# dmmiller612/sparktorch

Measured on AMD Instinct MI355X. Metric: samples_per_sec, higher is better.
Workload: dtype bf16; 1 GPU; model=mnist_mlp_784x256x256x10, global_batch=2097152, parallelism=dp1, optimizer=fused_adam, loss=cross_entropy_fused, hipgraph=False

## Files before the change

sparktorch_amd/ops/csrc/bindings.cpp:

```cpp

#include <torch/extension.h>

#include <c10/hip/HIPStream.h>
#include <hip/hip_runtime.h>

#include <cstdint>

typedef uint16_t bf16raw;

extern "C" {
hipError_t launch_fused_adam(float*, const float*, float*, float*, int64_t, float, float, float,
                             float, float, float, float, float, int, const int*, hipStream_t);
hipError_t launch_increment_i32(int*, hipStream_t);
hipError_t launch_fused_sgd(float*, const float*, float*, int64_t, float, float, float, float,
                            float, int, int, int, hipStream_t);
hipError_t launch_relu_bwd(const bf16raw*, const bf16raw*, bf16raw*, int64_t, hipStream_t);
hipError_t launch_bias_grad(const bf16raw*, float*, int, int, float*, int,
                            hipStream_t);
hipError_t launch_small_wgrad(const bf16raw*, const bf16raw*, float*, float*, int, int64_t, int,
                              int, hipStream_t);
hipError_t launch_pad_nhwc(const bf16raw*, bf16raw*, int, int, int, int, int, hipStream_t);
hipError_t launch_s2d_stem(const bf16raw*, bf16raw*, int, int, int, int, hipStream_t);
hipError_t launch_flip_w2d(const bf16raw*, bf16raw*, int, int, int, hipStream_t);
hipError_t launch_conv_implicit_fwd(const bf16raw*, const bf16raw*, const float*, bf16raw*, int,
                                    int, int, int, int, int, int, int, int, int, int, int, int,
                                    hipStream_t);
hipError_t launch_conv_implicit_wgrad(const bf16raw*, const bf16raw*, float*, int, int, int, int,
                                      int, int, int, int, int, int, float*, int, int,
                                      hipStream_t);
int conv_implicit_wgrad_slices(int, int);
hipError_t launch_cast_f64_f32(const double*, float*, int64_t, hipStream_t);
hipError_t launch_cast_f64_bf16(const double*, bf16raw*, int64_t, hipStream_t);
hipError_t launch_cast_f32_bf16(const float*, bf16raw*, int64_t, hipStream_t);
hipError_t launch_ce_fused(const bf16raw*, const int64_t*, float*, bf16raw*, int, int,
                           hipStream_t);
hipError_t launch_mse_fused(const bf16raw*, const bf16raw*, float*, bf16raw*, int64_t,
                            hipStream_t);
hipError_t launch_gemm_bf16(const void*, const void*, int, float*, bf16raw*, const float*, int,
                            int, int, int64_t, int64_t, int64_t, int64_t, int, int, float*, int,
                            hipStream_t);
hipError_t launch_gemm_bf16_mask(const void*, const void*, int, float*, bf16raw*, const float*,
                                 int, int, int, int64_t, int64_t, int64_t, int64_t, int, int,
                                 float*, int, const bf16raw*, hipStream_t);
int head_bwd_supported(int, int);
int linear_wgrad_stream_supported(int, int, int64_t);
int linear_wgrad_stream_can_run(int, int, int64_t);
hipError_t launch_linear_wgrad_stream(const bf16raw*, const bf16raw*, float*, float*, int64_t, int,
                                      int, int, int, hipStream_t);
int linear_fwd_stream_supported(int, int, int64_t);
int64_t linear_fwd_stream_min_rows();
hipError_t launch_linear_stream(const bf16raw*, const bf16raw*, bf16raw*, const float*,
                                const bf16raw*, int64_t, int, int, int, int, int, hipStream_t);
hipError_t launch_sample_gather(const void*, int, const void*, int, void*, void*, int*, const int*,
                                uint32_t, int64_t, int, int, int, int, hipStream_t);
hipError_t launch_head_bwd(const bf16raw*, const bf16raw*, const bf16raw*, bf16raw*, float*,
                           float*, int, int, int, int, int, hipStream_t);
hipError_t launch_bn_stats(const bf16raw*, float*, float*, float*, float*, float*, float*, int,
                           int, int64_t, float, float, int, hipStream_t);
hipError_t launch_bn_apply(const bf16raw*, const bf16raw*, bf16raw*, const float*, const float*,
                           const float*, const float*, int, int64_t, int64_t, int, hipStream_t);
hipError_t launch_bn_bwd_reduce(const bf16raw*, const bf16raw*, const bf16raw*, const float*,
                                const float*, float*, float*, int, int, int64_t, int,
                                hipStream_t);
hipError_t launch_bn_bwd_dx(const bf16raw*, const bf16raw*, const bf16raw*, const float*,
                            const float*, const float*, const float*, const float*, bf16raw*,
                            int, int64_t, int64_t, float, int, hipStream_t);
hipError_t launch_add_relu(const bf16raw*, const bf16raw*, bf16raw*, int64_t, hipStream_t);
hipError_t launch_maxpool_gen_fwd(const bf16raw*, bf16raw*, uint8_t*, int64_t, int, int, int,
                                  int, int, int, int, hipStream_t);
hipError_t launch_maxpool_gen_bwd(const bf16raw*, const uint8_t*, bf16raw*, int64_t, int, int,
                                  int, int, int, int, int, hipStream_t);
hipError_t launch_gap_fwd(const bf16raw*, bf16raw*, int64_t, int64_t, hipStream_t);
hipError_t launch_gap_bwd(const bf16raw*, bf16raw*, int64_t, int64_t, hipStream_t);
hipError_t launch_im2col_nhwc(const bf16raw*, bf16raw*, int, int, int, int, int, int, int, int,
                              int, int, int, int, int, hipStream_t);
hipError_t launch_col2im_nhwc(const bf16raw*, bf16raw*, int, int, int, int, int, int, int, int,
                              int, int, int, int, int, hipStream_t);
hipError_t launch_maxpool_nhwc_fwd(const bf16raw*, bf16raw*, uint8_t*, int, int, int, int, int,
                                   int, int, int, int, hipStream_t);
hipError_t launch_maxpool_nhwc_bwd(const bf16raw*, const uint8_t*, bf16raw*, int, int, int, int,
                                   int, int, int, int, int, hipStream_t);
hipError_t launch_gap_nhwc_fwd(const bf16raw*, bf16raw*, int, int, int64_t, hipStream_t);
hipError_t launch_gap_nhwc_bwd(const bf16raw*, bf16raw*, int, int, int64_t, hipStream_t);
hipError_t launch_bn_stats_nhwc(const bf16raw*, float*, float*, float*, float*, float*, float*,
                                int64_t, int, float, float, int, float*, int, hipStream_t);
hipError_t launch_bn_apply_nhwc(const bf16raw*, const bf16raw*, bf16raw*, const float*,
                                const float*, const float*, const float*, int, int64_t, int,
                                hipStream_t);
hipError_t launch_bn_bwd_reduce_nhwc(const bf16raw*, const bf16raw*, const bf16raw*,
// ... 417 lines not shown
    ip = idx_out->data_ptr<int>();
  }
  CHECK_HIP(launch_sample_gather(x.data_ptr(), (int)x.element_size(), yp, y_es, xb.data_ptr(), ybp,
                                 ip, step_dev.data_ptr<int>(), (uint32_t)(seed & 0xFFFFFFFFLL), n,
                                 (int)k, (int)F, (int)L, head_num_cus(), cur_stream()));
}

at::Tensor linear_head_bwd(at::Tensor dz_out, at::Tensor w, at::Tensor y_in, at::Tensor dw,
                           c10::optional<at::Tensor> db, int64_t max_blocks) {
  check_gpu_contig(dz_out, at::kBFloat16, "dz_out");
  check_gpu_contig(w, at::kBFloat16, "w");
  check_gpu_contig(y_in, at::kBFloat16, "y_in");
  check_gpu_contig(dw, at::kFloat, "dw");
  TORCH_CHECK(dz_out.dim() == 2 && w.dim() == 2 && y_in.dim() == 2);
  int64_t B = dz_out.size(0), C = dz_out.size(1), H = w.size(1);
  TORCH_CHECK(B >= 1 && B < (1LL << 31) && w.size(0) == C && y_in.size(0) == B &&
                  y_in.size(1) == H && dw.size(0) == C && dw.size(1) == H,
              "shape mismatch");
  TORCH_CHECK(head_bwd_ok(C, H), "linear_head_bwd: unsupported (C, H); use the per-layer route");
  float* dbp = nullptr;
  if (db.has_value()) {
    check_gpu_contig(*db, at::kFloat, "db");
    TORCH_CHECK(db->numel() == C);
    dbp = db->data_ptr<float>();
  }
  auto dz_in = at::empty({B, H}, y_in.options());
  TORCH_CHECK(((uintptr_t)y_in.data_ptr() & 15) == 0 && ((uintptr_t)dz_in.data_ptr() & 15) == 0,
              "linear_head_bwd wants 16-byte aligned activations");
  CHECK_HIP(launch_head_bwd((const bf16raw*)dz_out.data_ptr(), (const bf16raw*)w.data_ptr(),
                            (const bf16raw*)y_in.data_ptr(), (bf16raw*)dz_in.data_ptr(),
                            dw.data_ptr<float>(), dbp, (int)B, (int)C, (int)H, (int)max_blocks,
                            head_num_cus(), cur_stream()));
  return dz_in;
}


static bool small_wgrad_path(int64_t M, int64_t N, int64_t K) {
  return (K & 7) == 0 && N * K <= 2048 && N <= 64 && K <= 512 && M >= 65536;
}
static int small_wgrad_slices(int64_t M) {
  int64_t s = M / 4096;
  return (int)(s < 256 ? 256 : (s > 2048 ? 2048 : s));
}

at::Tensor linear_wgrad(at::Tensor dz, at::Tensor x, int64_t splitk) {
  check_gpu_contig(dz, at::kBFloat16, "dz");
  check_gpu_contig(x, at::kBFloat16, "x");
  int64_t B = dz.size(0), N = dz.size(1), K = x.size(1);
  TORCH_CHECK(x.size(0) == B, "shape mismatch");
  if (small_wgrad_path(B, N, K)) {
    auto dw = at::zeros({N, K}, x.options().dtype(at::kFloat));
    int S = small_wgrad_slices(B);
    auto scratch = at::empty({(int64_t)S * N * K}, x.options().dtype(at::kFloat));
    CHECK_HIP(launch_small_wgrad((const bf16raw*)dz.data_ptr(), (const bf16raw*)x.data_ptr(),
                                 dw.data_ptr<float>(), scratch.data_ptr<float>(), S, B, (int)N,
                                 (int)K, cur_stream()));
    return dw;
  }
  at::Tensor dw = splitk > 1 ? at::zeros({N, K}, x.options().dtype(at::kFloat))
                             : at::empty({N, K}, x.options().dtype(at::kFloat));
  CHECK_HIP(launch_gemm_bf16(dz.data_ptr(), x.data_ptr(),  0, dw.data_ptr<float>(),
                             nullptr, nullptr, (int)N, (int)K, (int)B,
                              1,  N,  K,  1, 0, (int)splitk,
                             nullptr, -1, cur_stream()));
  return dw;
}
// ... 527 lines not shown
  m.def("conv_implicit_wgrad", &conv_implicit_wgrad, "implicit-GEMM s1 conv weight grad",
        py::arg("dz"), py::arg("xP"), py::arg("KH"), py::arg("KW"), py::arg("splitk"),
        py::arg("slab"), py::arg("OHo") = -1, py::arg("OWo") = -1,
        py::arg("SH") = 1, py::arg("SW") = 1);
  m.def("cast_f64_f32", &cast_f64_f32);
  m.def("cast_f64_bf16", &cast_f64_bf16, "one-pass device Vector pack cast");
  m.def("cast_f32_bf16", &cast_f32_bf16);
  m.def("ce_fused", &ce_fused, "cross-entropy fwd+bwd fused");
  m.def("mse_fused", &mse_fused, "mse fwd+bwd fused");
  m.def("linear_fwd", &linear_fwd, "Y = X W^T (+bias)(+relu), MFMA", py::arg("x"), py::arg("w"),
        py::arg("bias"), py::arg("relu"), py::arg("allow_stream") = true);
  m.def("linear_dgrad", &linear_dgrad, "dX = dZ W, MFMA", py::arg("dz"), py::arg("w"),
        py::arg("allow_stream") = true);
  m.def("linear_fwd_stream_supported", &linear_fwd_stream_ok,
        "can the full-N streaming Linear kernel compute C[M, N] from a K-deep reduction",
        py::arg("N"), py::arg("K"), py::arg("M"));
  m.def("linear_fwd_stream_min_rows", &linear_stream_min_rows,
        "M from which linear_fwd / linear_dgrad(_relu) route supported shapes to it");
  m.def("set_linear_stream_min_rows", &set_linear_stream_min_rows,
        "override that M (tests); negative restores the measured one; returns the old setting",
        py::arg("rows"));
  m.def("linear_fwd_stream", &linear_fwd_stream,
        "Y = X W^T (+bias)(+relu) through the full-N streaming kernel, any M", py::arg("x"),
        py::arg("w"), py::arg("bias"), py::arg("relu"));
  m.def("linear_dgrad_stream", &linear_dgrad_stream,
        "dX = dZ W (* (y_prev > 0)) through the full-N streaming kernel, any M", py::arg("dz"),
        py::arg("w"), py::arg("y_prev") = py::none());
  m.def("linear_dgrad_relu", &linear_dgrad_relu, "dX = (dZ W) * (y_prev > 0), MFMA",
        py::arg("dz"), py::arg("w"), py::arg("y_prev"), py::arg("allow_stream") = true);
  m.def("head_bwd_supported", &head_bwd_ok, "does the one-pass head backward serve (C, H)");
  m.def("linear_head_bwd", &linear_head_bwd, "one-pass dz_in/dW/db of a small head on a ReLU layer",
        py::arg("dz_out"), py::arg("w"), py::arg("y_in"), py::arg("dw"), py::arg("db"),
        py::arg("max_blocks") = 0);
  m.def("linear_wgrad_stream_supported", &linear_wgrad_stream_ok,
        "is (No, Ki) at batch B routed to the batch-streaming wgrad");
  m.def("linear_wgrad_stream_can_run", &linear_wgrad_stream_runs,
        "can the batch-streaming wgrad compute (No, Ki, B) at all");
  m.def("linear_wgrad_stream", &linear_wgrad_stream,
        "dW (+ db) accumulated by the persistent batch-streaming kernel", py::arg("dz"),
        py::arg("x"), py::arg("dw"), py::arg("db") = py::none(), py::arg("max_blocks") = 0);
  m.def("linear_wgrad", &linear_wgrad, "dW = dZ^T X, MFMA split-K");
  m.def("linear_wgrad_into", &linear_wgrad_into, "dW accumulated into grad view");
  m.def("linear_wgrad_bias_into", &linear_wgrad_bias_into, "dW + db in one MFMA launch");
  m.def("bias_grad_into", &bias_grad_into, "db accumulated into grad view");
  m.def("matmul_bf16", &matmul_bf16, "generic bf16 MFMA GEMM");
  m.def("im2col", &im2col, "NCHW -> implicit-GEMM col matrix");
  m.def("col2im", &col2im, "col gradient -> NCHW input gradient");
  m.def("maxpool_fwd", &maxpool_fwd, "max_pool2d (kernel==stride) + argmax");
  m.def("maxpool_bwd", &maxpool_bwd, "max_pool2d backward scatter");
  m.def("dropout_apply", &dropout_apply, "counter-based dropout / dropout2d");
  m.def("bn_stats", &bn_stats, "BatchNorm2d training stats (mean, invstd) + running update");
  m.def("bn_apply", &bn_apply, "BN normalize+affine (+residual)(+relu)");
  m.def("bn_bwd_reduce", &bn_bwd_reduce, "BN backward: dbeta/dgamma accumulated in-place");
  m.def("bn_bwd_dx", &bn_bwd_dx, "BN backward input gradient");
  m.def("add_relu", &add_relu, "out = relu(a+b) (residual join)");
  m.def("maxpool_gen_fwd", &maxpool_gen_fwd, "general max_pool2d (stride/pad) + argmax");
  m.def("maxpool_gen_bwd", &maxpool_gen_bwd, "general max_pool2d backward (gather)");
  m.def("gap_fwd", &gap_fwd, "global average pool [B,C,H,W]->[B,C]");
  m.def("gap_bwd", &gap_bwd, "global average pool backward");
  m.def("im2col_nhwc", &im2col_nhwc, "BHWC -> implicit-GEMM col (vectorized over C)");
  m.def("col2im_nhwc", &col2im_nhwc, "col gradient -> BHWC input gradient");
  m.def("maxpool_nhwc_fwd", &maxpool_nhwc_fwd, "NHWC max_pool2d (stride/pad) + argmax");
  m.def("maxpool_nhwc_bwd", &maxpool_nhwc_bwd, "NHWC max_pool2d backward (gather)");
  m.def("gap_nhwc_fwd", &gap_nhwc_fwd, "NHWC global average pool -> [B,C]");
  m.def("gap_nhwc_bwd", &gap_nhwc_bwd, "NHWC global average pool backward");
  m.def("bn_stats_nhwc", &bn_stats_nhwc, "NHWC BN training stats + running update");
// ... 5 lines not shown
```

sparktorch_amd/ops/csrc/common.h:

```cpp
#pragma once

#include <hip/hip_runtime.h>

#include <cstdint>

#define WAVE 64

typedef uint16_t bf16raw;

__device__ __forceinline__ float bf16_to_f32(bf16raw h) {
  union {
    uint32_t u;
    float f;
  } c;
  c.u = ((uint32_t)h) << 16;
  return c.f;
}

__device__ __forceinline__ bf16raw f32_to_bf16(float f) {
  union {
    float f;
    uint32_t u;
  } c;
  c.f = f;
  uint32_t u = c.u;
  uint32_t rounding = 0x7fff + ((u >> 16) & 1);
  u += rounding;
  return (bf16raw)(u >> 16);
}

typedef float floatx4 __attribute__((ext_vector_type(4)));
typedef float floatx16 __attribute__((ext_vector_type(16)));
typedef short shortx8 __attribute__((ext_vector_type(8)));
typedef short shortx4 __attribute__((ext_vector_type(4)));

__host__ __device__ __forceinline__ int64_t ceil_div_i64(int64_t a, int64_t b) {
  return (a + b - 1) / b;
}

__host__ __device__ __forceinline__ uint32_t hash_u32(uint32_t a, uint32_t seed) {
  uint32_t h = a * 0x9E3779B9u + seed;
  h ^= h >> 16;
  h *= 0x85EBCA6Bu;
  h ^= h >> 13;
  h *= 0xC2B2AE35u;
  h ^= h >> 16;
  return h;
}

#define HIP_CHECK_LAUNCH()                                         \
  do {                                                             \
    hipError_t err_ = hipGetLastError();                           \
    if (err_ != hipSuccess) return err_;                           \
  } while (0)
```

sparktorch_amd/ops/csrc/head_bwd.hip:

```cpp

#include "common.h"

typedef shortx8 hfrag_t;

#define HEAD_THREADS 256
#define HEAD_CPAD 16

__host__ __device__ constexpr int head_rows(int H) { return H <= 256 ? 64 : 32; }

template <bool TR>
__device__ __forceinline__ hfrag_t head_tr_frag(const bf16raw* __restrict__ img, int stride,
                                                int xm, int rb, int q, int l15, int col0) {
  hfrag_t f;
  if (TR) {
    const int col = col0 + 4 * (l15 & 3);
#pragma unroll
    for (int jh = 0; jh < 2; ++jh) {
      const int row = rb + jh * 16 + q * 4 + (l15 >> 2);
      const bf16raw* p = img + row * stride + ((((col >> 3) ^ (row & xm)) << 3) | (col & 7));
      shortx4 v = __builtin_amdgcn_ds_read_tr16_b64_v4i16(
          (__attribute__((address_space(3))) shortx4*)p);
#pragma unroll
      for (int j = 0; j < 4; ++j) f[jh * 4 + j] = v[j];
    }
  } else {
    const int col = col0 + l15;
#pragma unroll
    for (int i = 0; i < 8; ++i) {
      const int row = rb + (i >> 2) * 16 + q * 4 + (i & 3);
      f[i] = (short)img[row * stride + ((((col >> 3) ^ (row & xm)) << 3) | (col & 7))];
    }
  }
  return f;
}

template <int H, bool TR>
__global__ __launch_bounds__(HEAD_THREADS, 2) void head_bwd_kernel(
    const bf16raw* __restrict__ dz_out, const bf16raw* __restrict__ w,
    const bf16raw* __restrict__ y_in, bf16raw* __restrict__ dz_in, float* __restrict__ dw,
    float* __restrict__ db, int B, int C) {
  constexpr int ROWS = head_rows(H);
  constexpr int SLOTS = H / 8;
  constexpr int XM = (SLOTS % 16 == 0) ? 15 : 7;
  constexpr int NP = H / 32;
  constexpr int PW = (NP + 3) / 4;
  constexpr int NCH = ROWS * H * 2 / 1024;
  constexpr int EPT = ROWS * HEAD_CPAD / HEAD_THREADS;
  static_assert(H % 64 == 0 && H <= 512, "unsupported H");

  __shared__ __attribute__((aligned(16))) bf16raw ys[2][ROWS * H];
  __shared__ __attribute__((aligned(16))) bf16raw dzs[2][ROWS * HEAD_CPAD];

  const int t = threadIdx.x;
  const int wid = t >> 6, lane = t & 63;
  const int l15 = lane & 15, q = lane >> 4;
  const int ntiles = (B + ROWS - 1) / ROWS;

  hfrag_t wf[PW][2];
#pragma unroll
  for (int pi = 0; pi < PW; ++pi) {
    const int p = wid + pi * 4;
#pragma unroll
    for (int e = 0; e < 2; ++e) {
      const int h = p * 32 + (l15 >> 2) * 8 + e * 4 + (l15 & 3);
#pragma unroll
      for (int i = 0; i < 8; ++i) {
        const int c = q * 8 + i;
        wf[pi][e][i] = (p < NP && c < C) ? (short)w[c * H + h] : (short)0;
      }
    }
  }
  hfrag_t ones;
#pragma unroll
  for (int i = 0; i < 8; ++i) ones[i] = (short)0x3F80;

  floatx4 accw[PW][2] = {};
  floatx4 accb = {0.f, 0.f, 0.f, 0.f};

  const int zrow = (t * EPT) / HEAD_CPAD, zc0 = (t * EPT) % HEAD_CPAD;
  bf16raw zr[EPT];
  auto load_dz = [&](int tile) {
    const int64_t gr = (int64_t)tile * ROWS + zrow;
#pragma unroll
    for (int j = 0; j < EPT; ++j)
      zr[j] = (gr < B && zc0 + j < C) ? dz_out[gr * C + zc0 + j] : (bf16raw)0;
  };
  auto write_dz = [&](int b) {
#pragma unroll
    for (int j = 0; j < EPT; ++j) dzs[b][zrow * HEAD_CPAD + zc0 + j] = zr[j];
  };
  auto dma_y = [&](int b, int tile) {
#pragma unroll
    for (int c = wid; c < NCH; c += 4) {
      const int o = c * 1024 + lane * 16;
      const int row = o / (H * 2);
      const int slot = ((o % (H * 2)) >> 4) ^ (row & XM);
      int64_t gr = (int64_t)tile * ROWS + row;
      if (gr > B - 1) gr = B - 1;
      const bf16raw* g = y_in + gr * H + slot * 8;
      __builtin_amdgcn_global_load_lds(
          (const __attribute__((address_space(1))) unsigned int*)g,
          (__attribute__((address_space(3))) unsigned int*)(ys[b] + c * 512), 16, 0, 0);
    }
  };

  int tile = blockIdx.x;
  int buf = 0;
  if (tile < ntiles) {
    dma_y(0, tile);
    load_dz(tile);
    write_dz(0);
  }
  for (; tile < ntiles; tile += gridDim.x) {
    __syncthreads();
    const int next = tile + gridDim.x;
    if (next < ntiles) {
      load_dz(next);
      dma_y(buf ^ 1, next);
    }
    const bf16raw* yb = ys[buf];
    const bf16raw* zb = dzs[buf];
    const int64_t row0 = (int64_t)tile * ROWS;

#pragma unroll
    for (int rf = 0; rf < ROWS / 16; ++rf) {
      const int row = rf * 16 + l15;
      hfrag_t bz = {};
      if (q < 2) bz = *(const hfrag_t*)&zb[row * HEAD_CPAD + q * 8];
#pragma unroll
      for (int pi = 0; pi < PW; ++pi) {
        const int p = wid + pi * 4;
        if (p < NP) {
          floatx4 z = {0.f, 0.f, 0.f, 0.f};
          floatx4 a0 = __builtin_amdgcn_mfma_f32_16x16x32_bf16(wf[pi][0], bz, z, 0, 0, 0);
          floatx4 a1 = __builtin_amdgcn_mfma_f32_16x16x32_bf16(wf[pi][1], bz, z, 0, 0, 0);
          const int slot = p * 4 + q;
          const shortx8 mk = *(const shortx8*)&yb[row * H + ((slot ^ (row & XM)) << 3)];
          shortx8 out;
#pragma unroll
          for (int j = 0; j < 4; ++j) {
            out[j] = bf16_to_f32((bf16raw)mk[j]) > 0.f ? (short)f32_to_bf16(a0[j]) : (short)0;
            out[4 + j] =
                bf16_to_f32((bf16raw)mk[4 + j]) > 0.f ? (short)f32_to_bf16(a1[j]) : (short)0;
          }
          if (row0 + row < B) *(shortx8*)(dz_in + (row0 + row) * H + slot * 8) = out;
        }
      }
    }

#pragma unroll
    for (int ks = 0; ks < ROWS / 32; ++ks) {
      const hfrag_t bz = head_tr_frag<TR>(zb, HEAD_CPAD, 0, ks * 32, q, l15, 0);
      if (wid == 0)
        accb = __builtin_amdgcn_mfma_f32_16x16x32_bf16(ones, bz, accb, 0, 0, 0);
#pragma unroll
      for (int pi = 0; pi < PW; ++pi) {
        const int p = wid + pi * 4;
        if (p < NP) {
#pragma unroll
          for (int e = 0; e < 2; ++e) {
            const hfrag_t ay = head_tr_frag<TR>(yb, H, XM, ks * 32, q, l15, p * 32 + e * 16);
            accw[pi][e] = __builtin_amdgcn_mfma_f32_16x16x32_bf16(ay, bz, accw[pi][e], 0, 0, 0);
          }
        }
      }
    }

    if (next < ntiles) write_dz(buf ^ 1);
    buf ^= 1;
  }

  if (l15 < C) {
#pragma unroll
    for (int pi = 0; pi < PW; ++pi) {
      const int p = wid + pi * 4;
      if (p < NP) {
#pragma unroll
        for (int e = 0; e < 2; ++e)
#pragma unroll
          for (int r = 0; r < 4; ++r)
            atomicAdd(dw + l15 * H + p * 32 + e * 16 + q * 4 + r, accw[pi][e][r]);
      }
    }
    if (db != nullptr && wid == 0 && q == 0) atomicAdd(db + l15, accb[0]);
  }
}

extern "C" int head_bwd_supported(int C, int H) {
  return C >= 1 && C <= HEAD_CPAD && (H == 64 || H == 128 || H == 256 || H == 512);
}

extern "C" hipError_t launch_head_bwd(const bf16raw* dz_out, const bf16raw* w,
                                      const bf16raw* y_in, bf16raw* dz_in, float* dw, float* db,
                                      int B, int C, int H, int max_blocks, int num_cus,
                                      hipStream_t stream) {
  if (!head_bwd_supported(C, H) || B < 1) return hipErrorInvalidValue;
  const int ntiles = (B + head_rows(H) - 1) / head_rows(H);
  int grid = 2 * (num_cus > 0 ? num_cus : 256);
  if (max_blocks > 0 && grid > max_blocks) grid = max_blocks;
  if (grid > ntiles) grid = ntiles;
#define HEAD_LAUNCH(HH)                                                                     \
  head_bwd_kernel<HH, true><<<dim3(grid), dim3(HEAD_THREADS), 0, stream>>>(dz_out, w, y_in, \
                                                                            dz_in, dw, db, B, C)
  switch (H) {
    case 64: HEAD_LAUNCH(64); break;
    case 128: HEAD_LAUNCH(128); break;
    case 256: HEAD_LAUNCH(256); break;
    default: HEAD_LAUNCH(512); break;
  }
#undef HEAD_LAUNCH
  HIP_CHECK_LAUNCH();
  return hipSuccess;
}
```

sparktorch_amd/ops/csrc/loss.hip:

```cpp

#include "common.h"


__global__ void ce_fused_kernel(const bf16raw* __restrict__ logits,
                                const int64_t* __restrict__ tgt, float* __restrict__ loss_out,
                                bf16raw* __restrict__ dlogits, int B, int C, float inv_B) {
  int64_t b = (int64_t)blockIdx.x * blockDim.x + threadIdx.x;
  float my_loss = 0.f;
  if (b < B) {
    const bf16raw* row = logits + b * C;
    bf16raw* drow = dlogits + b * C;
    float mx = -1e30f;
    for (int c = 0; c < C; ++c) mx = fmaxf(mx, bf16_to_f32(row[c]));
    float se = 0.f;
    for (int c = 0; c < C; ++c) se += __expf(bf16_to_f32(row[c]) - mx);
    float lse = __logf(se) + mx;
    int64_t t = tgt[b];
    my_loss = (lse - bf16_to_f32(row[t])) * inv_B;
    float inv_se = 1.f / se;
    for (int c = 0; c < C; ++c) {
      float p = __expf(bf16_to_f32(row[c]) - mx) * inv_se;
      if (c == (int)t) p -= 1.f;
      drow[c] = f32_to_bf16(p * inv_B);
    }
// ... 9 lines not shown
}

__global__ void ce_fused_wave_kernel(const bf16raw* __restrict__ logits,
                                     const int64_t* __restrict__ tgt,
                                     float* __restrict__ loss_out,
                                     bf16raw* __restrict__ dlogits, int B, int C, float inv_B) {
  int wave = threadIdx.x >> 6;
  int lane = threadIdx.x & 63;
  int64_t b = (int64_t)blockIdx.x * 4 + wave;
  if (b >= B) return;
  const bf16raw* row = logits + b * C;
  bf16raw* drow = dlogits + b * C;
  float mx = -1e30f;
  for (int c = lane; c < C; c += 64) mx = fmaxf(mx, bf16_to_f32(row[c]));
  for (int off = 32; off; off >>= 1) mx = fmaxf(mx, __shfl_xor(mx, off, 64));
  float se = 0.f;
  for (int c = lane; c < C; c += 64) se += __expf(bf16_to_f32(row[c]) - mx);
  for (int off = 32; off; off >>= 1) se += __shfl_xor(se, off, 64);
  int64_t t = tgt[b];
  float inv_se = 1.f / se;
  for (int c = lane; c < C; c += 64) {
    float p = __expf(bf16_to_f32(row[c]) - mx) * inv_se;
    if (c == (int)t) p -= 1.f;
    drow[c] = f32_to_bf16(p * inv_B);
  }
  if (lane == 0) {
    float my_loss = (__logf(se) + mx - bf16_to_f32(row[t])) * inv_B;
    atomicAdd(loss_out, my_loss);
  }
}

extern "C" hipError_t launch_ce_fused(const bf16raw* logits, const int64_t* tgt, float* loss_out,
                                      bf16raw* dlogits, int B, int C, hipStream_t stream) {
  if (C >= 128 || B <= 2048) {
    int grid = (int)ceil_div_i64(B, 4);
    ce_fused_wave_kernel<<<grid, 256, 0, stream>>>(logits, tgt, loss_out, dlogits, B, C,
                                                   1.0f / B);
  } else {
    int block = 256;
    int grid = (int)ceil_div_i64(B, block);
    ce_fused_kernel<<<grid, block, 0, stream>>>(logits, tgt, loss_out, dlogits, B, C, 1.0f / B);
  }
  HIP_CHECK_LAUNCH();
  return hipSuccess;
}


__global__ void mse_fused_kernel(const bf16raw* __restrict__ pred,
                                 const bf16raw* __restrict__ target, float* __restrict__ loss_out,
                                 bf16raw* __restrict__ dpred, int64_t n, float inv_n) {
  int64_t i = (int64_t)blockIdx.x * blockDim.x + threadIdx.x;
  int64_t stride = (int64_t)gridDim.x * blockDim.x;
  float my = 0.f;
  for (int64_t k = i; k < n; k += stride) {
    float d = bf16_to_f32(pred[k]) - bf16_to_f32(target[k]);
    my += d * d * inv_n;
    dpred[k] = f32_to_bf16(2.f * d * inv_n);
  }
  __shared__ float red[256];
  red[threadIdx.x] = my;
  __syncthreads();
  for (int s = blockDim.x / 2; s > 0; s >>= 1) {
    if (threadIdx.x < s) red[threadIdx.x] += red[threadIdx.x + s];
    __syncthreads();
  }
  if (threadIdx.x == 0 && red[0] != 0.f) atomicAdd(loss_out, red[0]);
}
// ... 11 lines not shown
```

sparktorch_amd/ops/functional.py:

```python

from __future__ import annotations

from typing import Optional

import torch
import torch.nn.functional as F

from sparktorch_amd import ops


def _choose_splitk(batch: int, n_out: int, k_in: int) -> int:
    base = -(-n_out // 128) * (-(-k_in) // 128)
    want = max(1, 2048 // max(1, base))
    max_by_rows = max(1, batch // 512)
    return int(min(want, max_by_rows, 512))


_WGRAD_STREAM = True
_WGRAD_STREAM_MIN_BATCH = None


def _wgrad_stream_ok(ext, dz: torch.Tensor, x: torch.Tensor) -> bool:
    if not _WGRAD_STREAM or dz.data_ptr() % 16 or x.data_ptr() % 16:
        return False
# ... 177 lines not shown
        b_direct = need_b and b_notify is not None and b.grad is not None
        dw_t = w.grad if w_direct else torch.zeros_like(w, dtype=torch.float32)
        db_t = None
        if need_b:
            db_t = b.grad if b_direct else torch.zeros_like(b, dtype=torch.float32)
        dz_prev = ext.linear_head_bwd(dz, wb, xin, dw_t, db_t, 0)
        if w_direct:
            w_notify()
        if b_direct:
            b_notify()
        return dz_prev, (None if w_direct else dw_t), (None if b_direct else db_t)


def hip_mlp_chain(x: torch.Tensor, layers) -> torch.Tensor:
    if x.is_cuda:
        if x.dtype != torch.bfloat16:
            x = x.to(torch.bfloat16)
        if not x.is_contiguous():
            x = x.contiguous()
        lead = x.shape[:-1]
        flat = []
        for w, b, _ in layers:
            flat += [w, b]
        relus = tuple(bool(r) for _, _, r in layers)
        y = _MLPChainFn.apply(x.reshape(-1, x.shape[-1]), relus, *flat)
        return y.view(*lead, y.shape[-1]) if x.dim() != 2 else y
    for w, b, relu in layers:
        x = F.linear(x, w, b)
        if relu:
            x = F.relu(x)
    return x


class _Conv2dFn(torch.autograd.Function):

    @staticmethod
    def forward(ctx, x, w, b, stride, padding, relu):
        ext = ops.ext()
        B, CI, H, W = x.shape
        CO, _, KH, KW = w.shape
        sh, sw = stride
        ph, pw = padding
        HO = (H + 2 * ph - KH) // sh + 1
        WO = (W + 2 * pw - KW) // sw + 1
        col = ext.im2col(x, KH, KW, sh, sw, ph, pw)
        w2d = w.reshape(CO, CI * KH * KW).contiguous()
        y2d = ext.linear_fwd(col, w2d, b, relu, allow_stream=False)
        ctx.save_for_backward(col, w2d, y2d)
        ctx.meta = (B, CI, H, W, CO, KH, KW, sh, sw, ph, pw, HO, WO, relu, b is not None)
        ctx.w_ref, ctx.b_ref = w, b
        return y2d.view(B, HO, WO, CO).permute(0, 3, 1, 2).contiguous()

    @staticmethod
    def backward(ctx, dy):
        ext = ops.ext()
        col, w2d, y2d = ctx.saved_tensors
        B, CI, H, W, CO, KH, KW, sh, sw, ph, pw, HO, WO, relu, has_bias = ctx.meta
        dy2d = dy.permute(0, 2, 3, 1).reshape(B * HO * WO, CO).contiguous()
        if dy2d.dtype != torch.bfloat16:
            dy2d = dy2d.to(torch.bfloat16)
        dz = ext.relu_bwd(dy2d, y2d) if relu else dy2d

        w, b = ctx.w_ref, ctx.b_ref
        dw = db = None
        sk = _choose_splitk(dz.shape[0], CO, col.shape[1])
        w_notify = getattr(w, "_bucket_notify", None)
# ... 607 lines not shown
```

sparktorch_amd/ops/modules.py:

```python

from __future__ import annotations

from typing import Optional

import torch
import torch.nn as nn

from sparktorch_amd.ops.functional import (
    hip_add_relu,
    hip_batch_norm2d,
    hip_batch_norm2d_nhwc,
    hip_conv2d,
    hip_conv2d_nhwc,
    hip_cross_entropy,
    hip_dropout,
    hip_global_avg_pool,
    hip_global_avg_pool_nhwc,
    hip_linear,
    hip_max_pool2d,
    hip_max_pool2d_nhwc,
    hip_mlp_chain,
    hip_relu,
    hip_mse,
)


class HipLinear(nn.Module):

    def __init__(self, in_features: int, out_features: int, bias: bool = True,
                 activation: Optional[str] = None):
        super().__init__()
        self.in_features = in_features
        self.out_features = out_features
        self.weight = nn.Parameter(torch.empty(out_features, in_features))
        self.bias = nn.Parameter(torch.zeros(out_features)) if bias else None
        self.activation = activation
        nn.init.kaiming_uniform_(self.weight, a=5 ** 0.5)

    @classmethod
    def from_linear(cls, lin: nn.Linear, activation: Optional[str] = None) -> "HipLinear":
        m = cls.__new__(cls)
        nn.Module.__init__(m)
        m.in_features = lin.in_features
        m.out_features = lin.out_features
        m.weight = lin.weight
        m.bias = lin.bias
        m.activation = activation
        return m

    def forward(self, x: torch.Tensor) -> torch.Tensor:
        return hip_linear(x, self.weight, self.bias, relu=self.activation == "relu")

    def extra_repr(self) -> str:
        return "in=%d, out=%d, act=%s" % (self.in_features, self.out_features, self.activation)
# ... 191 lines not shown
        self.fc = HipLinear(512, num_classes)

    def forward(self, x):
        if x.is_cuda and x.dtype != torch.bfloat16:
            x = x.to(torch.bfloat16)
        if x.dim() == 2:
            x = x.view(-1, 3, 224, 224)
        if self.layout == "nhwc":
            x = x.permute(0, 2, 3, 1).contiguous()
        x = self.bn1(self.conv1(x))
        x = self.maxpool(x)
        x = self.layers(x)
        return self.fc(self.gap(x))


class HipCrossEntropy(nn.Module):
    def forward(self, logits, target):
        return hip_cross_entropy(logits, target)


class HipMSE(nn.Module):
    def forward(self, pred, target):
        return hip_mse(pred, target)


class MnistMLPFused(nn.Module):

    def __init__(self, in_dim: int = 784, hidden: int = 256, classes: int = 10):
        super().__init__()
        self.fc1 = HipLinear(in_dim, hidden, activation="relu")
        self.fc2 = HipLinear(hidden, hidden, activation="relu")
        self.fc3 = HipLinear(hidden, classes, activation=None)

    def forward(self, x: torch.Tensor) -> torch.Tensor:
        return hip_mlp_chain(x, [(fc.weight, fc.bias, fc.activation == "relu")
                                 for fc in (self.fc1, self.fc2, self.fc3)])


def convert_model_for_mi355x(model: nn.Module) -> nn.Module:
    for name, child in model.named_children():
        cname = type(child).__name__
        if cname in ("Linear",) or isinstance(child, nn.Linear):
            setattr(model, name, HipLinear.from_linear(child))
        elif cname in ("Conv2d",) or isinstance(child, nn.Conv2d):
            try:
                setattr(model, name, HipConv2d.from_conv2d(child))
            except (ValueError, AttributeError):
                pass
        elif cname == "MaxPool2d" or isinstance(child, nn.MaxPool2d):
            ks, st, pd = child.kernel_size, child.stride, child.padding
            if isinstance(ks, int) and isinstance(st, (int, type(None))) and isinstance(pd, int) \
                    and child.dilation == 1 and not child.ceil_mode:
                setattr(model, name, HipMaxPool2d(ks, stride=st, padding=pd))
        elif cname == "BatchNorm2d" or isinstance(child, nn.BatchNorm2d):
            try:
                setattr(model, name, HipBatchNorm2d.from_batchnorm(child))
            except (ValueError, AttributeError):
                pass
        elif cname == "AdaptiveAvgPool2d" and child.output_size in (1, (1, 1)):
            setattr(model, name, HipGlobalAvgPool(keepdim=True))
        elif cname == "Dropout2d":
            setattr(model, name, HipDropout(p=child.p, channel_wise=True))
        elif cname == "Dropout":
            setattr(model, name, HipDropout(p=child.p, channel_wise=False))
        else:
            convert_model_for_mi355x(child)
    return model


# ... 8 lines not shown
```

sparktorch_amd/parallel/sync.py:

```python

from __future__ import annotations

import random
from typing import Any, Iterable, List, Optional

import numpy as np
import torch
import torch.distributed as dist

from sparktorch_amd.compat.barrier import get_barrier_context
from sparktorch_amd.parallel.buckets import FlatBuckets
from sparktorch_amd.parallel.rendezvous import (
    cleanup_stale_process_group,
    init_process_group_from_barrier,
    pick_device,
)
from sparktorch_amd.utils.data import handle_features, handle_features_device
from sparktorch_amd.utils.early_stopper import EarlyStopping
from sparktorch_amd.utils.sampling import DeviceMinibatchSampler
from sparktorch_amd.utils.trace import StepMetrics, trace_range
from sparktorch_amd.utils.serialize import (
    load_base_torch,
    load_torch_model,
    serialize_torch_obj,
# ... 39 lines not shown
                convert_model_for_mi355x,
            )

            self.model = convert_model_for_mi355x(self.model)
            self.criterion = convert_criterion_for_mi355x(self.criterion)
        self.world_size = (
            world_size
            if world_size is not None
            else (dist.get_world_size() if dist.is_initialized() else 1)
        )

        self.buckets = FlatBuckets(
            list(self.model.parameters()), bucket_cap_mb=bucket_cap_mb, world_size=self.world_size
        )
        self.buckets.register_hooks()

        from sparktorch_amd.ops.optim import fused_optimizer_for

        self.optimizer = fused_optimizer_for(torch_optimizer, self.buckets)
        self._torch_opt = None
        if self.optimizer is None:
            self._torch_opt = type(torch_optimizer)(
                self.model.parameters(), **torch_optimizer.defaults
            )

        self._graph = None
        self._graph_inputs = None
        self._sampled_graph = None
        self.compile_mode = compile_mode
        if compile_mode and compile_mode not in ("hipgraph",):
            self.model = torch.compile(self.model, mode=compile_mode)

    def _forward_backward(self, x: torch.Tensor, y: torch.Tensor) -> torch.Tensor:
        pred = self.model(x)
        loss = compute_loss(self.criterion, pred, y)
        loss.backward()
        return loss

    def train_step(self, x: torch.Tensor, y: torch.Tensor) -> float:
        if self.compile_mode == "hipgraph" and x.is_cuda:
            return self._train_step_graphed(x, y)
        self.buckets.zero_grad()
        loss = self._forward_backward(x, y)
        if self.optimizer is not None:
            self.buckets.finalize(average=False)
            self.optimizer.step(grad_scale=1.0 / self.world_size)
        else:
            self.buckets.finalize(average=True)
            self._torch_opt.step()
        return float(loss.detach())

    def _train_step_graphed(self, x: torch.Tensor, y: torch.Tensor) -> float:
        key = (tuple(x.shape), tuple(y.shape) if y is not None else None)
        if self._graph is None or self._graph_inputs[0] != key:
            if self.world_size > 1:
                raise RuntimeError(
                    "compileMode='hipgraph' currently supports world_size==1 "
                    "(collectives are not graph-captured)"
                )
            static_x = x.clone()
            static_y = y.clone() if y is not None else None
            snap_params = [b.flat_param.clone() for b in self.buckets.buckets]
            snap_buffers = {k: v.clone() for k, v in self.model.named_buffers()}
            snap_opt = None
            if self.optimizer is not None:
                sd = getattr(self.optimizer, "step_dev", None)
# ... 301 lines not shown
```

Measured before the change: 390.6 million samples/s.

## Fuse MLP head forward, cross-entropy and head backward into one kernel

Adds a head_ce kernel that computes head logits with MFMA, softmax cross-entropy, the loss reduction and the dlogits-driven backward (dz_in, dW, db) in a single pass over the last hidden activations. The MLP training step routes through a manual, autograd-free forward/backward chain when the criterion is HipCrossEntropy. This avoids writing and re-reading the logits and dlogits tensors and cuts separate kernel launches and autograd overhead. In exchange the code is more complex, uses inline barriers, and sums the loss with float atomics, so it is order-dependent.

After: 425.8 million samples/s, median of 6. 9.0% higher.

```diff
diff --git a/sparktorch_amd/ops/csrc/bindings.cpp b/sparktorch_amd/ops/csrc/bindings.cpp
--- a/sparktorch_amd/ops/csrc/bindings.cpp
+++ b/sparktorch_amd/ops/csrc/bindings.cpp
@@ -55,6 +55,8 @@
                                 uint32_t, int64_t, int, int, int, int, hipStream_t);
 hipError_t launch_head_bwd(const bf16raw*, const bf16raw*, const bf16raw*, bf16raw*, float*,
                            float*, int, int, int, int, int, hipStream_t);
+hipError_t launch_head_ce(const bf16raw*, const float*, const bf16raw*, const int64_t*, bf16raw*,
+                          float*, float*, float*, bf16raw*, int, int, int, int, int, hipStream_t);
 hipError_t launch_bn_stats(const bf16raw*, float*, float*, float*, float*, float*, float*, int,
                            int, int64_t, float, float, int, hipStream_t);
 hipError_t launch_bn_apply(const bf16raw*, const bf16raw*, bf16raw*, const float*, const float*,
@@ -538,6 +540,45 @@
                             dw.data_ptr<float>(), dbp, (int)B, (int)C, (int)H, (int)max_blocks,
                             head_num_cus(), cur_stream()));
   return dz_in;
+}
+
+std::tuple<at::Tensor, at::Tensor, at::Tensor> linear_head_ce(
+    at::Tensor y_in, at::Tensor w, c10::optional<at::Tensor> bias, at::Tensor target,
+    at::Tensor dw, c10::optional<at::Tensor> db, bool want_logits, int64_t max_blocks) {
+  check_gpu_contig(y_in, at::kBFloat16, "y_in");
+  check_gpu_contig(w, at::kBFloat16, "w");
+  check_gpu_contig(target, at::kLong, "target");
+  check_gpu_contig(dw, at::kFloat, "dw");
+  TORCH_CHECK(y_in.dim() == 2 && w.dim() == 2 && target.dim() == 1);
+  int64_t B = y_in.size(0), H = y_in.size(1), C = w.size(0);
+  TORCH_CHECK(B >= 1 && B < (1LL << 31) && w.size(1) == H && target.size(0) == B &&
+                  dw.dim() == 2 && dw.size(0) == C && dw.size(1) == H,
+              "shape mismatch");
+  TORCH_CHECK(head_bwd_ok(C, H), "linear_head_ce: unsupported (C, H); use the three-step route");
+  const float* bp = nullptr;
+  if (bias.has_value()) {
+    check_gpu_contig(*bias, at::kFloat, "bias");
+    TORCH_CHECK(bias->numel() == C);
+    bp = bias->data_ptr<float>();
+  }
+  float* dbp = nullptr;
+  if (db.has_value()) {
+    check_gpu_contig(*db, at::kFloat, "db");
+    TORCH_CHECK(db->numel() == C);
+    dbp = db->data_ptr<float>();
+  }
+  auto loss = at::empty({}, y_in.options().dtype(at::kFloat));
+  auto dz_in = at::empty({B, H}, y_in.options());
+  auto logits = want_logits ? at::empty({B, C}, y_in.options()) : at::empty({0}, y_in.options());
+  TORCH_CHECK(((uintptr_t)y_in.data_ptr() & 15) == 0 && ((uintptr_t)dz_in.data_ptr() & 15) == 0 &&
+                  ((uintptr_t)w.data_ptr() & 15) == 0,
+              "linear_head_ce wants 16-byte aligned activations and weights");
+  CHECK_HIP(launch_head_ce((const bf16raw*)w.data_ptr(), bp, (const bf16raw*)y_in.data_ptr(),
+                           target.data_ptr<int64_t>(), (bf16raw*)dz_in.data_ptr(),
+                           dw.data_ptr<float>(), dbp, loss.data_ptr<float>(),
+                           want_logits ? (bf16raw*)logits.data_ptr() : nullptr, (int)B, (int)C,
+                           (int)H, (int)max_blocks, head_num_cus(), cur_stream()));
+  return {loss, dz_in, logits};
 }
 
 
@@ -1131,6 +1172,10 @@
   m.def("linear_head_bwd", &linear_head_bwd, "one-pass dz_in/dW/db of a small head on a ReLU layer",
         py::arg("dz_out"), py::arg("w"), py::arg("y_in"), py::arg("dw"), py::arg("db"),
         py::arg("max_blocks") = 0);
+  m.def("linear_head_ce", &linear_head_ce,
+        "head forward + cross-entropy + one-pass head backward: (loss, dz_in, logits)",
+        py::arg("y_in"), py::arg("w"), py::arg("bias"), py::arg("target"), py::arg("dw"),
+        py::arg("db"), py::arg("want_logits") = false, py::arg("max_blocks") = 0);
   m.def("linear_wgrad_stream_supported", &linear_wgrad_stream_ok,
         "is (No, Ki) at batch B routed to the batch-streaming wgrad");
   m.def("linear_wgrad_stream_can_run", &linear_wgrad_stream_runs,
diff --git a/sparktorch_amd/ops/csrc/common.h b/sparktorch_amd/ops/csrc/common.h
--- a/sparktorch_amd/ops/csrc/common.h
+++ b/sparktorch_amd/ops/csrc/common.h
@@ -48,7 +48,9 @@
   return h;
 }
 
-#define HIP_CHECK_LAUNCH()                                         \
+#define CE_WAVE_MAX_B 2048
+
+#define HIP_CHECK_LAUNCH()                                        \
   do {                                                             \
     hipError_t err_ = hipGetLastError();                           \
     if (err_ != hipSuccess) return err_;                           \
diff --git a/sparktorch_amd/ops/csrc/head_bwd.hip b/sparktorch_amd/ops/csrc/head_bwd.hip
--- a/sparktorch_amd/ops/csrc/head_bwd.hip
+++ b/sparktorch_amd/ops/csrc/head_bwd.hip
@@ -34,11 +34,13 @@
   return f;
 }
 
-template <int H, bool TR>
-__global__ __launch_bounds__(HEAD_THREADS, 2) void head_bwd_kernel(
+template <int H, bool TR, bool CE>
+__device__ __forceinline__ void head_tiles(
     const bf16raw* __restrict__ dz_out, const bf16raw* __restrict__ w,
     const bf16raw* __restrict__ y_in, bf16raw* __restrict__ dz_in, float* __restrict__ dw,
-    float* __restrict__ db, int B, int C) {
+    float* __restrict__ db, int B, int C, const float* __restrict__ bias,
+    const int64_t* __restrict__ tgt, float* __restrict__ loss, bf16raw* __restrict__ logits_out,
+    float inv_B) {
   constexpr int ROWS = head_rows(H);
   constexpr int SLOTS = H / 8;
   constexpr int XM = (SLOTS % 16 == 0) ? 15 : 7;
@@ -49,7 +51,7 @@
   static_assert(H % 64 == 0 && H <= 512, "unsupported H");
 
   __shared__ __attribute__((aligned(16))) bf16raw ys[2][ROWS * H];
-  __shared__ __attribute__((aligned(16))) bf16raw dzs[2][ROWS * HEAD_CPAD];
+  __shared__ __attribute__((aligned(16))) bf16raw dzs[CE ? 1 : 2][ROWS * HEAD_CPAD];
 
   const int t = threadIdx.x;
   const int wid = t >> 6, lane = t & 63;
@@ -76,6 +78,25 @@
 
   floatx4 accw[PW][2] = {};
   floatx4 accb = {0.f, 0.f, 0.f, 0.f};
+
+  hfrag_t wk[CE ? H / 32 : 1];
+  float bias_c = 0.f, lsum = 0.f;
+  int tg[4] = {0, 0, 0, 0};
+  if (CE) {
+#pragma unroll
+    for (int ks = 0; ks < H / 32; ++ks) {
+      wk[ks] = hfrag_t{};
+      if (l15 < C) wk[ks] = *(const hfrag_t*)&w[l15 * H + ks * 32 + q * 8];
+    }
+    if (bias != nullptr && l15 < C) bias_c = bias[l15];
+  }
+  auto load_tgt = [&](int tile) {
+    if (wid < ROWS / 16) {
+      const int64_t gr = (int64_t)tile * ROWS + wid * 16 + q * 4;
+#pragma unroll
+      for (int r = 0; r < 4; ++r) tg[r] = (gr + r < B) ? (int)tgt[gr + r] : 0;
+    }
+  };
 
   const int zrow = (t * EPT) / HEAD_CPAD, zc0 = (t * EPT) % HEAD_CPAD;
   bf16raw zr[EPT];
@@ -108,19 +129,101 @@
   int buf = 0;
   if (tile < ntiles) {
     dma_y(0, tile);
-    load_dz(tile);
-    write_dz(0);
+    if (CE) {
+      load_tgt(tile);
+    } else {
+      load_dz(tile);
+      write_dz(0);
+    }
   }
   for (; tile < ntiles; tile += gridDim.x) {
-    __syncthreads();
+    if (CE)
+      asm volatile("s_waitcnt vmcnt(0) lgkmcnt(0)\n\ts_barrier" ::: "memory");
+    else
+      __syncthreads();
     const int next = tile + gridDim.x;
-    if (next < ntiles) {
+    const bf16raw* yb = ys[buf];
+    bf16raw* zb = dzs[CE ? 0 : buf];
+    const int64_t row0 = (int64_t)tile * ROWS;
+    if (CE) {
+      int tc[4];
+#pragma unroll
+      for (int r = 0; r < 4; ++r) tc[r] = tg[r];
+      constexpr bool EARLY = H <= 256;
+      const bool fwd_wave = wid < ROWS / 16;
+      const int arow = wid * 16 + l15;
+      hfrag_t ay[H / 32];
+      if (EARLY && fwd_wave) {
+#pragma unroll
+        for (int ks = 0; ks < H / 32; ++ks)
+          ay[ks] = *(const hfrag_t*)&yb[arow * H + (((ks * 4 + q) ^ (arow & XM)) << 3)];
+      }
+      if (next < ntiles) {
+        dma_y(buf ^ 1, next);
+        load_tgt(next);
+      }
+      if (fwd_wave) {
+#pragma clang fp reassociate(off)
+        floatx4 lg = {0.f, 0.f, 0.f, 0.f};
+#pragma unroll
+        for (int ks = 0; ks < H / 32; ++ks) {
+          if (!EARLY)
+            ay[ks] = *(const hfrag_t*)&yb[arow * H + (((ks * 4 + q) ^ (arow & XM)) << 3)];
+          lg = __builtin_amdgcn_mfma_f32_16x16x32_bf16(ay[ks], wk[ks], lg, 0, 0, 0);
+        }
+        constexpr int RG = H <= 256 ? 4 : 1;
+#pragma unroll
+        for (int r0 = 0; r0 < 4; r0 += RG) {
+          bf16raw xb[RG];
+          float x[RG], mx[RG], e[RG], se[RG];
+#pragma unroll
+          for (int j = 0; j < RG; ++j) {
+            xb[j] = f32_to_bf16(bias != nullptr ? lg[r0 + j] + bias_c : lg[r0 + j]);
+            x[j] = bf16_to_f32(xb[j]);
+            mx[j] = l15 < C ? fmaxf(-1e30f, x[j]) : -1e30f;
+          }
+#pragma unroll
+          for (int off = 8; off; off >>= 1)
+#pragma unroll
+            for (int j = 0; j < RG; ++j) mx[j] = fmaxf(mx[j], __shfl_xor(mx[j], off, 16));
+#pragma unroll
+          for (int j = 0; j < RG; ++j) e[j] = l15 < C ? __expf(x[j] - mx[j]) : 0.f;
+          if (B <= CE_WAVE_MAX_B) {
+#pragma unroll
+            for (int j = 0; j < RG; ++j) se[j] = e[j];
+#pragma unroll
+            for (int off = 8; off; off >>= 1)
+#pragma unroll
+              for (int j = 0; j < RG; ++j) se[j] += __shfl_xor(se[j], off, 16);
+          } else {
+#pragma unroll
+            for (int j = 0; j < RG; ++j) se[j] = 0.f;
+            for (int c = 0; c < C; ++c)
+#pragma unroll
+              for (int j = 0; j < RG; ++j) se[j] += __shfl(e[j], c, 16);
+          }
+#pragma unroll
+          for (int j = 0; j < RG; ++j) {
+            const int r = r0 + j;
+            const int lrow = wid * 16 + q * 4 + r;
+            const bool live = row0 + lrow < B;
+            const float xt = __shfl(x[j], tc[r] & 15, 16);
+            const float inv_se = 1.f / se[j];
+            const float p =
+                l15 == tc[r] ? __builtin_fmaf(e[j], inv_se, -1.f) : e[j] * inv_se;
+            zb[lrow * HEAD_CPAD + l15] =
+                (live && l15 < C) ? f32_to_bf16(p * inv_B) : (bf16raw)0;
+            if (live && l15 == 0) lsum += (__logf(se[j]) + mx[j] - xt) * inv_B;
+            if (logits_out != nullptr && live && l15 < C)
+              logits_out[(row0 + lrow) * C + l15] = xb[j];
+          }
+        }
+      }
+      asm volatile("s_waitcnt lgkmcnt(0)\n\ts_barrier" ::: "memory");
+    } else if (next < ntiles) {
       load_dz(next);
       dma_y(buf ^ 1, next);
     }
-    const bf16raw* yb = ys[buf];
-    const bf16raw* zb = dzs[buf];
-    const int64_t row0 = (int64_t)tile * ROWS;
 
 #pragma unroll
     for (int rf = 0; rf < ROWS / 16; ++rf) {
@@ -166,8 +269,22 @@
       }
     }
 
-    if (next < ntiles) write_dz(buf ^ 1);
+    if (!CE && next < ntiles) write_dz(buf ^ 1);
     buf ^= 1;
+  }
+
+  if (CE) {
+    __shared__ float lred[HEAD_THREADS / 64];
+#pragma unroll
+    for (int off = 32; off; off >>= 1) lsum += __shfl_xor(lsum, off, 64);
+    if (lane == 0) lred[wid] = lsum;
+    __syncthreads();
+    if (t == 0) {
+      float s = 0.f;
+#pragma unroll
+      for (int i = 0; i < HEAD_THREADS / 64; ++i) s += lred[i];
+      if (s != 0.f) atomicAdd(loss, s);
+    }
   }
 
   if (l15 < C) {
@@ -184,6 +301,25 @@
     }
     if (db != nullptr && wid == 0 && q == 0) atomicAdd(db + l15, accb[0]);
   }
+}
+
+template <int H, bool TR>
+__global__ __launch_bounds__(HEAD_THREADS, 2) void head_bwd_kernel(
+    const bf16raw* __restrict__ dz_out, const bf16raw* __restrict__ w,
+    const bf16raw* __restrict__ y_in, bf16raw* __restrict__ dz_in, float* __restrict__ dw,
+    float* __restrict__ db, int B, int C) {
+  head_tiles<H, TR, false>(dz_out, w, y_in, dz_in, dw, db, B, C, nullptr, nullptr, nullptr,
+                           nullptr, 0.f);
+}
+
+template <int H>
+__global__ __launch_bounds__(HEAD_THREADS, 2) void head_ce_kernel(
+    const bf16raw* __restrict__ w, const float* __restrict__ bias,
+    const bf16raw* __restrict__ y_in, const int64_t* __restrict__ tgt,
+    bf16raw* __restrict__ dz_in, float* __restrict__ dw, float* __restrict__ db,
+    float* __restrict__ loss, bf16raw* __restrict__ logits_out, int B, int C, float inv_B) {
+  head_tiles<H, true, true>(nullptr, w, y_in, dz_in, dw, db, B, C, bias, tgt, loss, logits_out,
+                            inv_B);
 }
 
 extern "C" int head_bwd_supported(int C, int H) {
@@ -212,3 +348,28 @@
   HIP_CHECK_LAUNCH();
   return hipSuccess;
 }
+
+extern "C" hipError_t launch_head_ce(const bf16raw* w, const float* bias, const bf16raw* y_in,
+                                     const int64_t* tgt, bf16raw* dz_in, float* dw, float* db,
+                                     float* loss, bf16raw* logits_out, int B, int C, int H,
+                                     int max_blocks, int num_cus, hipStream_t stream) {
+  if (!head_bwd_supported(C, H) || B < 1) return hipErrorInvalidValue;
+  const int ntiles = (B + head_rows(H) - 1) / head_rows(H);
+  int grid = 2 * (num_cus > 0 ? num_cus : 256);
+  if (max_blocks > 0 && grid > max_blocks) grid = max_blocks;
+  if (grid > ntiles) grid = ntiles;
+  hipError_t err = hipMemsetAsync(loss, 0, sizeof(float), stream);
+  if (err != hipSuccess) return err;
+#define HEAD_CE_LAUNCH(HH)                                                    \
+  head_ce_kernel<HH><<<dim3(grid), dim3(HEAD_THREADS), 0, stream>>>(          \
+      w, bias, y_in, tgt, dz_in, dw, db, loss, logits_out, B, C, 1.0f / B)
+  switch (H) {
+    case 64: HEAD_CE_LAUNCH(64); break;
+    case 128: HEAD_CE_LAUNCH(128); break;
+    case 256: HEAD_CE_LAUNCH(256); break;
+    default: HEAD_CE_LAUNCH(512); break;
+  }
+#undef HEAD_CE_LAUNCH
+  HIP_CHECK_LAUNCH();
+  return hipSuccess;
+}
diff --git a/sparktorch_amd/ops/csrc/loss.hip b/sparktorch_amd/ops/csrc/loss.hip
--- a/sparktorch_amd/ops/csrc/loss.hip
+++ b/sparktorch_amd/ops/csrc/loss.hip
@@ -65,7 +65,7 @@
 
 extern "C" hipError_t launch_ce_fused(const bf16raw* logits, const int64_t* tgt, float* loss_out,
                                       bf16raw* dlogits, int B, int C, hipStream_t stream) {
-  if (C >= 128 || B <= 2048) {
+  if (C >= 128 || B <= CE_WAVE_MAX_B) {
     int grid = (int)ceil_div_i64(B, 4);
     ce_fused_wave_kernel<<<grid, 256, 0, stream>>>(logits, tgt, loss_out, dlogits, B, C,
                                                    1.0f / B);
diff --git a/sparktorch_amd/ops/functional.py b/sparktorch_amd/ops/functional.py
--- a/sparktorch_amd/ops/functional.py
+++ b/sparktorch_amd/ops/functional.py
@@ -233,6 +233,78 @@
     return x
 
 
+_HEAD_CE_FUSION = True
+
+
+def _head_ce_ok(ext, w: torch.Tensor) -> bool:
+    return _HEAD_CE_FUSION and _head_bwd_ok(ext, w)
+
+
+def linear_head_ce(y_in, w, bias, target, dw, db=None, want_logits: bool = False,
+                   max_blocks: int = 0):
+    ext = ops.ext()
+    if _head_ce_ok(ext, w):
+        loss, dz_in, logits = ext.linear_head_ce(y_in, w, bias, target, dw, db, want_logits,
+                                                 max_blocks)
+        return loss, dz_in, (logits if want_logits else None)
+    logits = ext.linear_fwd(y_in, w, bias, False, _LINEAR_STREAM)
+    loss, dlogits = ext.ce_fused(logits, target)
+    dz_in = linear_head_bwd(dlogits, w, y_in, dw, db, max_blocks)
+    return loss, dz_in, (logits if want_logits else None)
+
+
+def _grad_is_direct(p) -> bool:
+    return (p.requires_grad and p.grad is not None and p.grad.dtype == torch.float32
+            and p.grad.is_contiguous() and getattr(p, "_bucket_notify", None) is not None)
+
+
+def mlp_chain_ce_supported(x: torch.Tensor, layers) -> bool:
+    if not (x.is_cuda and not x.requires_grad and len(layers) >= 2):
+        return False
+    if layers[-1][2] or not layers[-2][2]:
+        return False
+    for w, b, _ in layers:
+        if w.dtype != torch.float32 or not _grad_is_direct(w):
+            return False
+        if b is not None and not _grad_is_direct(b):
+            return False
+    w = layers[-1][0]
+    return bool(_HEAD_CE_FUSION and _HEAD_FUSION
+                and ops.ext().head_bwd_supported(w.shape[0], w.shape[1]))
+
+
+@torch.no_grad()
+def mlp_chain_ce_step(x: torch.Tensor, layers, target: torch.Tensor) -> torch.Tensor:
+    ext = ops.ext()
+    if x.dtype != torch.bfloat16:
+        x = x.to(torch.bfloat16)
+    if not x.is_contiguous():
+        x = x.contiguous()
+    x = x.reshape(-1, x.shape[-1])
+    target = target.flatten().long().contiguous()
+    n = len(layers)
+    acts, wbs = [x], []
+    for w, b, relu in layers[:-1]:
+        wbs.append(ext.cast_f32_bf16(w))
+        acts.append(ext.linear_fwd(acts[-1], wbs[-1], b, bool(relu), _LINEAR_STREAM))
+    w, b, _ = layers[-1]
+    loss, dz, _ = linear_head_ce(acts[-1], ext.cast_f32_bf16(w), b, target, w.grad,
+                                 b.grad if b is not None else None)
+    w._bucket_notify()
+    if b is not None:
+        b._bucket_notify()
+    for i in range(n - 2, -1, -1):
+        w, b, _ = layers[i]
+        dz_prev = None
+        if i > 0 and layers[i - 1][2]:
+            dz_prev = ext.linear_dgrad_relu(dz, wbs[i], acts[i], _LINEAR_STREAM)
+        elif i > 0:
+            dz_prev = ext.linear_dgrad(dz, wbs[i], _LINEAR_STREAM)
+        _linear_param_grads(ext, dz, acts[i], w, b, True, b is not None)
+        dz = dz_prev
+    return loss
+
+
 class _Conv2dFn(torch.autograd.Function):
 
     @staticmethod
diff --git a/sparktorch_amd/ops/modules.py b/sparktorch_amd/ops/modules.py
--- a/sparktorch_amd/ops/modules.py
+++ b/sparktorch_amd/ops/modules.py
@@ -20,6 +20,8 @@
     hip_max_pool2d,
     hip_max_pool2d_nhwc,
     hip_mlp_chain,
+    mlp_chain_ce_step,
+    mlp_chain_ce_supported,
     hip_relu,
     hip_mse,
 )
@@ -277,9 +279,18 @@
         self.fc2 = HipLinear(hidden, hidden, activation="relu")
         self.fc3 = HipLinear(hidden, classes, activation=None)
 
+    def _layers(self):
+        return [(fc.weight, fc.bias, fc.activation == "relu")
+                for fc in (self.fc1, self.fc2, self.fc3)]
+
     def forward(self, x: torch.Tensor) -> torch.Tensor:
-        return hip_mlp_chain(x, [(fc.weight, fc.bias, fc.activation == "relu")
-                                 for fc in (self.fc1, self.fc2, self.fc3)])
+        return hip_mlp_chain(x, self._layers())
+
+    def ce_step_supported(self, x: torch.Tensor) -> bool:
+        return mlp_chain_ce_supported(x, self._layers())
+
+    def ce_step(self, x: torch.Tensor, target: torch.Tensor) -> torch.Tensor:
+        return mlp_chain_ce_step(x, self._layers(), target)
 
 
 def convert_model_for_mi355x(model: nn.Module) -> nn.Module:
diff --git a/sparktorch_amd/parallel/sync.py b/sparktorch_amd/parallel/sync.py
--- a/sparktorch_amd/parallel/sync.py
+++ b/sparktorch_amd/parallel/sync.py
@@ -95,6 +95,15 @@
             self.model = torch.compile(self.model, mode=compile_mode)
 
     def _forward_backward(self, x: torch.Tensor, y: torch.Tensor) -> torch.Tensor:
+        if (
+            self.native
+            and type(self.criterion).__name__ == "HipCrossEntropy"
+            and (not self.compile_mode or self.compile_mode == "hipgraph")
+            and y is not None
+            and hasattr(self.model, "ce_step_supported")
+            and self.model.ce_step_supported(x)
+        ):
+            return self.model.ce_step(x, y)
         pred = self.model(x)
         loss = compute_loss(self.criterion, pred, y)
         loss.backward()
```
